# nsbuitrago/parasail-rs

Hardware: AMD Instinct MI355X
Metric: GCUPS (cell updates/s) local-affine SW, 1M 150x150 pairs, 1/2/4/8 GPUs (higher is better)
Workload: dtype int16

## Files before the change

### parasail-rs_amd/csrc/pmx_api.hip

```cpp
#include "pmx_common.h"
#include "pmx_switches.h"
#include <chrono>
#include <future>
#include "pmx_matrices.h"

#include <cctype>
#include <dlfcn.h>
#include <cstdarg>
#include <cstdio>
#include <cstdlib>
#include <cstring>
#include <algorithm>
#include <atomic>
#include <condition_variable>
#include <memory>
#include <mutex>
#include <string>
#include <system_error>
#include <thread>
#include <unordered_map>
#include <utility>
#include <vector>

static const PmxSwitchDoc g_switches[] = {
// ... 376 lines not shown
{
    if (!matrix) return;
    MatrixBox *b = nullptr;
    {
        std::lock_guard<std::mutex> lk(g_mx_mutex);
        auto it = g_boxes.find(matrix);
        if (it == g_boxes.end()) return;
        b = it->second; g_boxes.erase(it);
    }
    devcache_drop(matrix);
    delete b;
}

struct DevMat { PmxDevMatrix d; int16_t *scores; uint8_t *mapper; uint64_t hash; int rows; };
static std::mutex g_dev_mutex;
static std::unordered_map<uint64_t, DevMat> g_devmats;

static uint64_t mat_hash(const parasail_matrix_t *m)
{
    uint64_t h = 1469598103934665603ULL;
    auto mix = [&](int v) { h ^= (uint32_t)v; h *= 1099511628211ULL; };
    const size_t cells = (size_t)m->length * m->size;
    for (size_t i = 0; i < cells; ++i) mix(m->matrix[i]);
    for (int i = 0; i < 256; ++i) mix(m->mapper[i]);
    mix(m->size); mix(m->length); mix(m->type);
    return h;
}

static void devcache_drop(const parasail_matrix_t *m)
{
    std::lock_guard<std::mutex> lk(g_dev_mutex);
    for (auto it = g_devmats.begin(); it != g_devmats.end();) {
        if ((it->first >> 8) == ((uint64_t)(uintptr_t)m)) {
            (void)hipFree(it->second.scores); (void)hipFree(it->second.mapper);
            it = g_devmats.erase(it);
        } else ++it;
    }
}

static int get_devmat(const parasail_matrix_t *m, DevMat *out)
{
    if (!m || !m->matrix || !m->mapper || m->size <= 0 || m->size > 255) { set_err("bad matrix"); return -1; }
    if (m->max > 32767 || m->min < -32768) { set_err("matrix scores do not fit int16"); return -1; }
    int dev = 0; HIP_OR_RET(hipGetDevice(&dev));
    const uint64_t key = ((uint64_t)(uintptr_t)m << 8) | (uint64_t)(dev & 0xFF);
    const uint64_t h = mat_hash(m);
    std::lock_guard<std::mutex> lk(g_dev_mutex);
    auto it = g_devmats.find(key);
    if (it != g_devmats.end() && it->second.hash == h) { *out = it->second; return 0; }
    if (it != g_devmats.end()) { (void)hipFree(it->second.scores); (void)hipFree(it->second.mapper); g_devmats.erase(it); }
    const size_t cells = (size_t)m->length * m->size;
    std::vector<int16_t> s16(cells); std::vector<uint8_t> map8(256);
    for (size_t i = 0; i < cells; ++i) s16[i] = (int16_t)m->matrix[i];
    for (int i = 0; i < 256; ++i) {
        int v = m->mapper[i];
        if (v < 0 || v >= m->size) v = m->size - 1;
        map8[i] = (uint8_t)v;
    }
    DevMat dm; dm.hash = h; dm.rows = m->length;
    HIP_OR_RET(hipMalloc(&dm.scores, cells * 2));
    HIP_OR_RET(hipMalloc(&dm.mapper, 256));
    HIP_OR_RET(hipMemcpy(dm.scores, s16.data(), cells * 2, hipMemcpyHostToDevice));
    HIP_OR_RET(hipMemcpy(dm.mapper, map8.data(), 256, hipMemcpyHostToDevice));
    dm.d.scores = dm.scores; dm.d.mapper = dm.mapper; dm.d.msize = m->size; dm.d.min = m->min; dm.d.max = m->max;
    dm.d.pssm = m->type == PARASAIL_MATRIX_TYPE_PSSM ? 1 : 0; dm.d.rows = dm.d.pssm ? m->length : m->size;
    g_devmats[key] = dm;
    *out = dm;
    return 0;
}

enum {
    F_NW = 1 << 0, F_SG = 1 << 1, F_SW = 1 << 2, F_SATURATED = 1 << 6, F_BANDED = 1 << 7,
    F_SCAN = 1 << 10, F_STRIPED = 1 << 11, F_DIAG = 1 << 12, F_BLOCKED = 1 << 13,
    F_STATS = 1 << 16, F_TABLE = 1 << 17, F_ROWCOL = 1 << 18, F_TRACE = 1 << 19,
    F_BITS_8 = 1 << 20, F_BITS_16 = 1 << 21, F_BITS_32 = 1 << 22, F_BITS_64 = 1 << 23
};

struct PmxPendQueue;
struct parasail_result {
    int score, end_query, end_ref, flag;
    int matches, similar, length;
    int qlen, rlen;
    int *tables[4];
    int *rows[4];
    int *cols[4];
    int8_t *trace;
    struct PmxPendRef *pending;
};
static void pend_resolve(const parasail_result_t *r);
#define RESOLVE(r) do { if (__atomic_load_n(&(r)->pending, __ATOMIC_ACQUIRE)) pend_resolve(r); } while (0)

extern "C" {
int parasail_result_get_score(const parasail_result_t *r) { RESOLVE(r); return r->score; }
int parasail_result_get_end_query(const parasail_result_t *r) { RESOLVE(r); return r->end_query; }
int parasail_result_get_end_ref(const parasail_result_t *r) { RESOLVE(r); return r->end_ref; }
int parasail_result_get_matches(const parasail_result_t *r) { RESOLVE(r); return r->matches; }
int parasail_result_get_similar(const parasail_result_t *r) { RESOLVE(r); return r->similar; }
int parasail_result_get_length(const parasail_result_t *r) { RESOLVE(r); return r->length; }
// ... 740 lines not shown
        return "pmx_general_kernel";
    }
    if (fast_sw_eligible(cfg) && cfg->matrix->size <= PMX_MAX_FAST_MSIZE && max_qlen <= 2048 && max_rlen <= 60000)
        return "pmx_sw16_kernel";
    if ((cfg->mode == PMX_MODE_NW || cfg->mode == PMX_MODE_SG) && (cfg->want & ~PMX_WANT_SORTED) == 0 &&
        cfg->matrix->type == PARASAIL_MATRIX_TYPE_SQUARE && cfg->open >= cfg->extend && max_qlen <= 2048 &&
        cfg->matrix->size < PMX_MAX_FAST_MSIZE)
        return "pmx_nwsg16_kernel";
    if ((cfg->mode == PMX_MODE_NW || cfg->mode == PMX_MODE_SG) && (cfg->want & ~PMX_WANT_SORTED) == PMX_WANT_STATS && cfg->width != 8 &&
        cfg->matrix->type == PARASAIL_MATRIX_TYPE_SQUARE && cfg->open >= cfg->extend && cfg->extend >= 1 &&
        max_qlen <= 1024 && cfg->matrix->size < PMX_MAX_FAST_MSIZE)
        return "pmx_stats16_kernel";
    if ((cfg->want & ~PMX_WANT_SORTED) == 0 && cfg->matrix->type == PARASAIL_MATRIX_TYPE_SQUARE && cfg->matrix->size <= 64 &&
        (cfg->mode == PMX_MODE_SW || (cfg->width != 8 && cfg->width != 16)))
        return "pmx_long32_kernel";
    return "pmx_general_kernel";
}

struct Scratch { void *p = nullptr; size_t cap = 0; int dev = -1; };
enum { SCR_BOUND = 0, SCR_TRACE = 1, SCR_OPS = 2, SCR_SORT = 3, SCR_RETRY = 4,
       SCR_HQ = 5, SCR_HR = 6, SCR_HQO = 7, SCR_HRO = 8, SCR_HREC = 9, SCR_HST = 10,
       SCR_CIG = 11,
       SCR_HTEXT = 12, SCR_HTOFF = 13,
       SCR_HQ2 = 14, SCR_HR2 = 15,
       SCR_LONG = 16,
       SCR_SEL = 17,
       SCR_SRCH = 18, SCR_GREF = 19,
       SCR_PAIRS = 20, SCR_PGEN = 21,
       SCR_PUP = 22, SCR_PREC = 23, SCR_PST = 24,
       SCR_PSRCH = 25,
       SCR_PHIT = 26,
       SCR_PTOPK = 27,
       SCR_PTHIT = 28,
       SCR_SLOTS = 29 };
static thread_local Scratch g_scratch_pool[SCR_SLOTS];
static int scratch_reserve(size_t bytes, void **out, int slot = SCR_BOUND)
{
    Scratch &g_scratch = g_scratch_pool[slot];
    int dev = 0; HIP_OR_RET(hipGetDevice(&dev));
    if (g_scratch.dev != dev || g_scratch.cap < bytes) {
        if (g_scratch.p) {
            if (g_scratch.dev != dev) (void)hipSetDevice(g_scratch.dev);
            (void)hipFree(g_scratch.p);
            if (g_scratch.dev != dev) (void)hipSetDevice(dev);
        }
        g_scratch.p = nullptr; g_scratch.cap = 0; g_scratch.dev = dev;
        HIP_OR_RET(hipMalloc(&g_scratch.p, bytes ? bytes : 16));
        g_scratch.cap = bytes;
    }
    *out = g_scratch.p;
    return 0;
}

static thread_local const char *g_last_kernel = "";
extern "C" const char *pmx_last_kernel(void) { return g_last_kernel; }
static const char *nwsg_trace_kernel_name(const char *walk)
{
    static thread_local char name[160];
    snprintf(name, sizeof name, "%s%s", pmx_nwsg_trace_name(), walk);
    return name;
}


static PmxGeneralArgs general_args(const pmx_config_t *cfg, const DevMat &dm, int64_t n,
                                   const uint8_t *d_qbuf, const int64_t *d_qoff, int q_shared,
                                   const uint8_t *d_rbuf, const int64_t *d_roff, int32_t max_rlen)
{
    PmxGeneralArgs a; memset(&a, 0, sizeof a);
    a.qbuf = d_qbuf; a.qoff = q_shared ? nullptr : d_qoff; a.shared_qlen = q_shared;
    a.rbuf = d_rbuf; a.roff = d_roff; a.n = n; a.max_rlen = max_rlen;
    a.scores = dm.d.scores; a.mapper = dm.d.mapper; a.msize = dm.d.msize; a.mat_rows = dm.d.rows; a.pssm = dm.d.pssm;
    a.mode = cfg->mode; a.sg_flags = cfg->sg_flags; a.open = cfg->open; a.ext = cfg->extend;
    a.band = -1; a.bits = cfg->width;
    return a;
}

static int general_batch(const PmxGeneralArgs &t, bool want_stats, hipStream_t st, const char *what = "general kernel launch failed")
{
    const int64_t n = t.n;
    const size_t stride = (size_t)8 * t.max_rlen;
    const bool fits = pmx_general_lds_fits(t.mat_rows, t.msize, t.max_rlen);
    const size_t rs_stride = fits ? 0 : (((size_t)t.max_rlen + 8 + 15) & ~(size_t)15);
    const size_t per_pair = stride * sizeof(int32_t) + rs_stride;
// ... 402 lines not shown
                            int32_t max_qlen, int32_t max_rlen,
                            pmx_record_t *d_out, pmx_stats_t *d_stats_out, void *stream,
                            int q_shared_wild )
{
    if (check_cfg(cfg)) return -1;
    if (n <= 0) return 0;
    if (max_qlen <= 0 || max_rlen <= 0) { set_err("max_qlen / max_rlen must be positive"); return -1; }
    if ((cfg->want & PMX_WANT_STATS) && !d_stats_out) { set_err("stats requested without a stats buffer"); return -1; }
    if (cfg->want & PMX_WANT_CIGAR) { set_err("use pmx_align_batch_cigar for CIGAR output"); return -1; }
    if (pssm_batch_check(cfg->matrix, max_qlen, max_qlen)) return -1;
    DevMat dm;
    if (get_devmat(cfg->matrix, &dm)) return -1;
    hipStream_t st = (hipStream_t)stream;
    PmxBatch b = {d_qbuf, d_qoff, d_rbuf, d_roff, n, max_qlen, max_rlen, q_shared, nullptr, nullptr, nullptr, 0, 0};
    const int want = cfg->want & ~PMX_WANT_SORTED;
    if (dm.d.pssm && want == 0) { b.q_shared = max_qlen; q_shared_wild = 0; }
    if ((cfg->want & PMX_WANT_SORTED) && n >= 64 && n < (1LL << 32)) {
        void *scr = nullptr;
        if (scratch_reserve(pmx_sort_scratch_bytes(n), &scr, SCR_SORT)) return -1;
        const int rc = pmx_build_length_perm(d_roff, n, scr, &b.perm, st);
        if (rc < 0) { set_err("length sort failed (%d)", rc); return rc; }
    }
    long long long_min_cells = 250000;
    if (const char *e = pmx_env("PMX_LONG_MIN_CELLS")) long_min_cells = atoll(e);
    if (want == 0 && ((n <= 16 && max_qlen >= 512 && (long long)max_qlen * max_rlen >= long_min_cells) || max_qlen > 2048)) {
        const int rc = long_batch(cfg, dm, b, n, max_qlen, max_rlen, d_out, st);
        if (rc <= 0) return rc;
    }
    if (fast_sw_eligible(cfg)) {
        b.q_has_wildcard = b.q_shared ? q_shared_wild : 0;
        b.sat_above = cfg->width == 8 ? 127 : 0;
        if (n >= 4096 && n < (1LL << 32) && !b.q_has_wildcard) {
            void *scr = nullptr;
            if (scratch_reserve(((size_t)n + 1) * sizeof(unsigned), &scr, SCR_RETRY)) return -1;
            b.retry_count = (int *)scr;
            b.retry_list = (unsigned *)scr + 1;
        }
        const int rc = pmx_launch_sw16(b, dm.d, cfg->open, cfg->extend, d_out, st, &g_last_kernel);
        if (rc < 0) { set_err("sw16 launch failed: %s", hipGetErrorString((hipError_t)(-rc))); return rc; }
        if (rc == 0) return promote_overflowed(cfg, dm, b, d_out, st);
    }
    if (q_shared && want == PMX_WANT_STATS && cfg->width != 8 && (cfg->matrix->type == PARASAIL_MATRIX_TYPE_SQUARE || dm.d.pssm) &&
        (cfg->mode == PMX_MODE_NW || cfg->mode == PMX_MODE_SG) && (n >= 512 || pmx_env("PMX_STATS_BY_TRACE"))) {
        const int rc = stats_by_trace_shared(cfg, dm, b, d_out, d_stats_out, st);
        if (rc <= 0) return rc;
    }
    if (upload_wait(INT64_MAX, st, 0)) return -1;
    if (want == PMX_WANT_STATS && cfg->width != 8 && cfg->matrix->type == PARASAIL_MATRIX_TYPE_SQUARE) {
        auto launched = [](int rc, const char *what) {
            if (rc < 0) set_err("%s launch failed: %s", what, hipGetErrorString((hipError_t)(-rc)));
            return rc;
        };
        int rc = dm.d.msize <= 8 ? stats_by_trace_pairs(cfg, dm, b, d_out, d_stats_out, st) : 1;
        if (rc == 1)
            rc = launched(pmx_launch_stats16p(b, dm.d, cfg->mode, cfg->sg_flags, cfg->open, cfg->extend, d_out, d_stats_out, st, &g_last_kernel), "stats16p");
        if (rc == 1 && dm.d.msize > 8 && (max_rlen <= 1024 || pmx_env("PMX_STATS_BY_TRACE_ANY")))
            rc = stats_by_trace_pairs(cfg, dm, b, d_out, d_stats_out, st);
        if (rc == 1)
            rc = launched(pmx_launch_stats16(b, dm.d, cfg->mode, cfg->sg_flags, cfg->open, cfg->extend, d_out, d_stats_out, st, &g_last_kernel), "stats16");
        if (rc <= 0) return rc;
    }
    if ((cfg->mode == PMX_MODE_NW || cfg->mode == PMX_MODE_SG) && want == 0 && (cfg->width != 8 || !pmx_env("PMX_NWSG8_GENERAL")) &&
        (cfg->matrix->type == PARASAIL_MATRIX_TYPE_SQUARE || dm.d.pssm)) {
        b.track8 = cfg->width == 8;
        if (dm.d.msize <= 5 && n >= 2048 && !q_shared) {
            void *scr = nullptr;
            if (scratch_reserve(((size_t)n / 2 + 16) * sizeof(int), &scr, SCR_RETRY)) return -1;
            b.blockflag = (int *)scr;
        }
// ... 2698 lines not shown
```

### parasail-rs_amd/csrc/pmx_common.h

```cpp
#pragma once
#include <hip/hip_runtime.h>
#include <stdint.h>
#include "../../include/parasail_amd.h"
#include "../../include/pmx_conventions.h"

#define PMX_MAX_FAST_MSIZE 32

int pmx_ensure_lds_attr(const void *kernel, int bytes = 160 * 1024);

struct PmxDevMatrix {
    const int16_t *scores;
    const uint8_t *mapper;
    int msize;
    int min, max;
    int pssm;
    int rows;
};

struct PmxBatch {
    const uint8_t *qbuf; const int64_t *qoff;
    const uint8_t *rbuf; const int64_t *roff;
    int64_t n;
    int max_qlen, max_rlen;
    int q_shared;
    const unsigned *perm;
    unsigned *retry_list;
    int *retry_count;
    int q_has_wildcard;
    int sat_above;
    int track8;
    int *blockflag;
};
#define PMX_FLAG_RETRY16 4
#define PMX_FLAG_STRAND1 0x40000000

int pmx_launch_sw16(const PmxBatch &b, const PmxDevMatrix &m, int open, int ext,
                    pmx_record_t *d_out, hipStream_t stream, const char **kernel_name);

int pmx_sw16_trace_plan(const PmxBatch &b, const PmxDevMatrix &m, int open, int ext, int *variant, int *Tmax, size_t *trace_bytes);
int pmx_launch_sw16_trace(int variant, const PmxBatch &b, const PmxDevMatrix &m, int open, int ext,
                          pmx_record_t *d_out, uint32_t *tbuf, int Tmax, hipStream_t stream);

int pmx_nwsgv_bias(const PmxBatch &b, const PmxDevMatrix &m, int open, int ext, int rowx = 0, int shape_rows = 0 );
int pmx_launch_stats16p(const PmxBatch &b, const PmxDevMatrix &m, int mode, int sg_flags, int open, int ext,
                        pmx_record_t *d_out, pmx_stats_t *d_stats, hipStream_t stream, const char **kernel_name);

int pmx_nwsgv_trace_plan(const PmxBatch &b, const PmxDevMatrix &m, int mode, int open, int ext,
                         int *variant, int *Tmax, size_t *trace_bytes);
int pmx_launch_nwsgv_trace(int variant, const PmxBatch &b, const PmxDevMatrix &m, int mode, int sg_flags, int open, int ext,
                           pmx_record_t *d_out, uint32_t *tbuf, int Tmax, hipStream_t stream);
// ... 212 lines not shown
```

### parasail-rs_amd/csrc/pmx_sw16.hip

```cpp
#include "pmx_common.h"
#include "pmx_switches.h"
#include "pmx_pk16.h"
#include <cstdlib>

__device__ __forceinline__ v2s pk_adds(v2s a, v2s b) { return __builtin_elementwise_add_sat(a, b); }
__device__ __forceinline__ v2s pk_subs(v2s a, v2s b) { return __builtin_elementwise_sub_sat(a, b); }
__device__ __forceinline__ v2s pk_max(v2s a, v2s b) { return __builtin_elementwise_max(a, b); }

#ifndef PMX_SHARE_PERIOD
#define PMX_SHARE_PERIOD 16
#endif
#ifndef PMX_SW16_FUSED_HANDOFF
#define PMX_SW16_FUSED_HANDOFF 1
#endif
#define PMX_SW16_RETRY_BLOCKS 1024
#define FLOOR2 0x80008000

template <int G, int R, int VAR>
__global__ __launch_bounds__(64, (VAR == 6 && R <= 20) ? 4 : 1)
void pmx_sw16_kernel(const uint8_t *__restrict__ qbuf, const int64_t *__restrict__ qoff,
                     const uint8_t *__restrict__ rbuf, const int64_t *__restrict__ roff,
                     long long n, const int16_t *__restrict__ gmat, const uint8_t *__restrict__ gmap,
                     int msize, int open, int ext, int RP ,
                     int q_shared ,
                     int limit ,
                     const unsigned *__restrict__ perm,
                     const int *__restrict__ n_dev ,
                     unsigned *__restrict__ retry_list, int *__restrict__ retry_count ,
                     int sat_above ,
                     uint32_t *__restrict__ tbuf, int Tmax ,
                     pmx_record_t *__restrict__ out)
{
    if (n_dev) n = *n_dev;
    if ((long long)blockIdx.x * (2 * (64 / G)) >= n) return;
    constexpr bool LOOPED = VAR == 5;
    constexpr bool M3 = VAR >= 1;
    constexpr bool V2 = VAR >= 2;
    constexpr bool PT = VAR == 6;
    constexpr bool TR = VAR == 7;
    static_assert(!TR || R == 16, "trace: four packed planes of 4 rows");
    constexpr bool FETCH = VAR == 8;
    constexpr bool U8 = VAR == 3 || VAR == 5 || PT || TR || FETCH;
    constexpr bool SK = VAR >= 4;
    constexpr int EB = U8 ? 1 : 2;
    constexpr int WR = U8 ? 4 : 2;
    constexpr int RS = (R + WR - 1) / WR * WR;
    constexpr int QP = G * RS;
    constexpr int QP2 = QP / 2;
    constexpr int SLOTS = 64 / G;
    constexpr int NP = 2 * SLOTS;
    extern __shared__ __attribute__((aligned(16))) unsigned char lds[];

    long long pair0 = (long long)blockIdx.x * NP;
    do {
    int lane = threadIdx.x;
    if (LOOPED) {
        asm volatile("" : "+v"(lane));
        __syncthreads();
    }
    constexpr bool IL = G == 8 && VAR != 7;
    const int g = IL ? (lane % 16) / 2 : lane % G;
    const int slot = IL ? (lane / 16) * 2 + (lane & 1) : lane / G;
    const int PROF_STRIDE = PT ? 0 : msize * QP * EB;

    constexpr int PT_TABS = 32;
    int16_t *prof = reinterpret_cast<int16_t *>(lds);
    unsigned char *rsym = lds + (PT ? PT_TABS : NP * PROF_STRIDE + QP * EB);
    int16_t *mat = reinterpret_cast<int16_t *>(rsym + (FETCH ? 0 : NP * RP));
    unsigned char *map0 = reinterpret_cast<unsigned char *>(mat + msize * msize);
    long long *ptab = reinterpret_cast<long long *>(map0 + (PT ? 0 : 256) + ((8 - ((msize * msize * 2) & 7)) & 7));

    typedef __attribute__((address_space(3))) int *lds_int;
    auto tab_at = [](int byte) -> int { return *(lds_int)(uintptr_t)byte; };
    unsigned char *tabq = reinterpret_cast<unsigned char *>(ptab + 5 * NP);
    unsigned *wildf = reinterpret_cast<unsigned *>(tabq + 256);
    unsigned *ownmask = wildf + SLOTS;
    constexpr int OWN0 = 4 * (RS / 4 - 1), OWNN = OWN0 + R + 1;
    static_assert(!PT || OWNN <= 64, "one lane per mask");
    unsigned char *map = PT ? reinterpret_cast<unsigned char *>(ownmask + OWNN) : map0;
    static_assert(!PT || (G % 4 == 0 && RS % 4 == 0), "perm-table staging works on dwords");
    constexpr int PADF = PT ? G : G - 1;

    for (int i = lane; i < msize * msize; i += 64) mat[i] = gmat[i];
    if (PT) {
        const unsigned c4 = reinterpret_cast<const unsigned *>(gmap)[lane];
        reinterpret_cast<unsigned *>(map)[lane] = c4 << 2;
        reinterpret_cast<unsigned *>(tabq)[lane] = c4 + (c4 & 0x04040404u) * 6u;
    } else
        for (int i = lane; i < 256; i += 64) map[i] = gmap[i];
    if (PT && lane < SLOTS) wildf[lane] = 0;
    if (PT && lane < OWNN) ownmask[lane] = (unsigned)((0xFFFFFFFFull << (8 * min(max(lane - OWN0, 0), 4))) >> 32);
    if (lane < NP) {
        long long pos = pair0 + lane; if (pos >= n) pos = n - 1;
        const long long pi = perm ? (long long)perm[pos] : pos;
        const long long qb = q_shared ? 0 : qoff[pi], rb = roff[pi];
        ptab[5 * lane + 0] = qb;
        ptab[5 * lane + 1] = q_shared ? q_shared : (qoff[pi + 1] - qb);
        ptab[5 * lane + 2] = rb;
        ptab[5 * lane + 3] = roff[pi + 1] - rb;
        ptab[5 * lane + 4] = (pair0 + lane < n) ? pi : -1;
    }
    __syncthreads();
    const uint8_t *qbase = qbuf;
    const uint8_t *rbase = rbuf;

    int max_rlen = 0;
#pragma unroll
    for (int p = 0; p < NP; ++p) max_rlen = max(max_rlen, (int)ptab[5 * p + 3]);
    constexpr int UB = NP < 8 ? NP : 8;
    for (int p0 = 0; p0 < ((FETCH || PT) ? 0 : NP); p0 += UB) {
        for (int j0 = 0; j0 < RP; j0 += 64) {
            const int j = j0 + lane, jr = j - (G - 1);
            unsigned char raw[UB]; bool ok[UB];
#pragma unroll
            for (int u = 0; u < UB; ++u) {
                const int p = p0 + u;
                ok[u] = jr >= 0 && jr < (int)ptab[5 * p + 3];
                raw[u] = ok[u] ? rbase[ptab[5 * p + 2] + jr] : (unsigned char)0;
            }
            if (j < RP) {
#pragma unroll
                for (int u = 0; u < UB; ++u) {
                    const int p = p0 + u;
                    rsym[p * RP + j] = ok[u] ? map[raw[u]] : (unsigned char)((NP - p) * msize);
// ... 80 lines not shown
            const int ql = (int)ptab[5 * p + 1];
            const uint8_t *qp = qbase + ptab[5 * p + 0];
            const int p0 = 2 * rp, p1 = 2 * rp + 1;
            const int k0 = p0 % RS, k1 = p1 % RS;
            const int row0 = (p0 / RS) * R + k0, row1 = (p1 / RS) * R + k1;
            v0[u] = item < NP * QP2 && k0 < R && row0 < ql; v1[u] = item < NP * QP2 && k1 < R && row1 < ql;
            r0[u] = v0[u] ? qp[row0] : (unsigned char)0;
            r1[u] = v1[u] ? qp[row1] : (unsigned char)0;
        }
#pragma unroll
        for (int u = 0; u < QB; ++u) {
            const int item = (it0 + u) * 64 + lane;
            if (it0 + u < QITEMS && item < NP * QP2) {
                const int p = item / QP2, rp = item - p * QP2;
                const int q0 = v0[u] ? map[r0[u]] : -1;
                const int q1 = v1[u] ? map[r1[u]] : -1;
                for (int sym = 0; sym < msize; ++sym) {
                    const int s0 = ((q0 < 0) ? 0 : mat[q0 * msize + sym]) + (V2 ? open : 0);
                    const int s1 = ((q1 < 0) ? 0 : mat[q1 * msize + sym]) + (V2 ? open : 0);
                    if (U8) {
                        reinterpret_cast<unsigned short *>(lds + p * PROF_STRIDE + sym * QP)[rp] =
                            (unsigned short)((s0 & 0xFF) | ((s1 & 0xFF) << 8));
                    } else {
                        int *pp = reinterpret_cast<int *>(prof) + p * (PROF_STRIDE / 4) + rp;
                        pp[sym * QP2] = (s0 & 0xFFFF) | (s1 << 16);
                    }
                }
            }
        }
    }
    if (!PT) {
        for (int idx = lane; idx < QP * EB / 4; idx += 64)
            reinterpret_cast<int *>(lds + NP * PROF_STRIDE)[idx] = V2 ? 0 : FLOOR2;
    }
    if (PT) {
        if (lane <= msize) {
            int v = 0;
            if (lane < msize)
                for (int k = 0; k < 4 && k < msize; ++k) v |= ((mat[k * msize + lane] + open) & 0xFF) << (8 * k);
            ((lds_int)(uintptr_t)0)[lane] = v;
        }
    }
    __syncthreads();

    const int pA = 2 * slot, pB = 2 * slot + 1;
    const unsigned char *profA = lds + pA * PROF_STRIDE + g * (RS * EB);
    const unsigned char *profB = lds + pB * PROF_STRIDE + g * (RS * EB);
    constexpr int SS = PT ? 2 : 1;
    const unsigned char *rsA = PT ? rsym + slot * 2 * RP + 2 * (PADF - g) : rsym + pA * RP + (G - 1) - g;
    const unsigned char *rsB = PT ? rsA + 1 : rsym + pB * RP + (G - 1) - g;
    const int SYMSTRIDE = QP * EB;

    const v2s vOpen = PK((open & 0xFFFF) | (open << 16));
    const v2s vExt = PK((ext & 0xFFFF) | (ext << 16));
    constexpr int ZERO2 = M3 ? PK16_SW_BIAS2 : FLOOR2;
    const v2s vZero = PK(ZERO2);

    v2s HA[R], HB[R], E[R], Hsave[R];
    const int skew0 = SK ? (((G - g) * ext) & 0xFFFF) * 0x00010001 : 0;
    const v2s vC = PK(I32(vOpen) - I32(vExt));
    const v2s vInitH = V2 ? PK(ZERO2 - I32(vOpen) + skew0) : vZero;
#pragma unroll
    for (int k = 0; k < R; ++k) { HA[k] = vInitH; E[k] = V2 ? vInitH : (M3 ? PK(0) : vZero); Hsave[k] = vZero; }
    constexpr bool FUSED = SK && PMX_SW16_FUSED_HANDOFF && group_shift_fusable<G, IL>;
    if (FUSED) HB[R - 1] = PK(I32(vInitH) - I32(vExt));
    v2s best = PK(ZERO2 + skew0 - (SK ? I32(vC) : 0));
    int bestcol = g * 0x00010001;
    int vprev = 0, fake = 0;
    const int Zv0 = ZERO2 + skew0 + I32(vExt);
    const int HNEUTRAL = V2 ? ZERO2 - I32(vOpen) : ZERO2;
    int Hout = SK ? Zv0 - I32(vExt) - I32(vOpen) : HNEUTRAL, Fout = SK ? Zv0 - I32(vExt) : ZERO2;
    int Zprev = Zv0 - I32(vExt);
    int extV = I32(vExt);
    if (FUSED) asm("" : "+v"(extV));
// ... 156 lines not shown
        const v2s nbest = pk_max3(best, PK(fresh), PK(old));
        fake |= pk_lt(best, nbest);
        best = nbest;
        vprev = v;
    };
    const unsigned char *rcur = rsA;
    for (int t = 0;; t += 2) {
        if (SK && G > 1 && (t & (SHP - 1)) == 0 && t) share_bound();
        load_scores(nsA, nsB, w1a, w1b);
        if (FETCH) { nsA = symA_of(m2a); nsB = symB_of(m2b); fetch(t + 4, m2a, m2b); }
        else if (PT) { nsA = rcur[2 * SS]; nsB = rcur[2 * SS + 1]; asm("" : "+v"(nsA), "+v"(nsB)); }
        else { nsA = rsA[t + 2]; nsB = rsB[t + 2]; }
        __builtin_amdgcn_sched_barrier(0);
        step(HA, HB, w0a, w0b, t);
        __builtin_amdgcn_sched_barrier(0);
        if (t + 1 < T) {
            load_scores(nsA, nsB, w0a, w0b);
            if (FETCH) { nsA = symA_of(m3a); nsB = symB_of(m3b); fetch(t + 5, m3a, m3b); }
            else if (PT) { nsA = rcur[3 * SS]; nsB = rcur[3 * SS + 1]; asm("" : "+v"(nsA), "+v"(nsB)); rcur += 2 * SS; }
            else { nsA = rsA[t + 3]; nsB = rsB[t + 3]; }
            __builtin_amdgcn_sched_barrier(0);
            step(HB, HA, w1a, w1b, t + 1);
            __builtin_amdgcn_sched_barrier(0);
        } else
            asm("" : "=v"(Hout));
        if (t + 2 >= T) break;
    }

    unsigned long long keyA, keyB;
    {
        const int bA = (short)(I32(best) & 0xFFFF), bB = (short)(I32(best) >> 16);
        const unsigned stA = bestcol & 0xFFFF, stB = (unsigned)bestcol >> 16;
        const unsigned cA = stA - g, cB = stB - g;
        const int tA = SK ? bA - (T - (int)stA) * ext : bA, tB = SK ? bB - (T - (int)stB) * ext : bB;
        int kA = 0, kB = 0;
#pragma unroll
        for (int k = R - 1; k >= 0; --k) {
            if ((short)(I32(Hsave[k]) & 0xFFFF) == tA) kA = k;
            if ((short)(I32(Hsave[k]) >> 16) == tB) kB = k;
        }
        const int unskew = SK ? (G - g + T) * ext - (open - ext) : 0;
        const unsigned sA = (unsigned)(bA - unskew - (M3 ? PK16_SW_BIAS : -32768)), sB = (unsigned)(bB - unskew - (M3 ? PK16_SW_BIAS : -32768));
        const unsigned rA = g * R + kA, rB = g * R + kB;
        keyA = ((unsigned long long)sA << 32) | ((0xFFFFu - cA) << 16) | (0xFFFFu - rA);
        keyB = ((unsigned long long)sB << 32) | ((0xFFFFu - cB) << 16) | (0xFFFFu - rB);
        if (fake & 0xFFFF) keyA = 0;
        if (fake >> 16) keyB = 0;
    }
#pragma unroll
    for (int off = G / 2; off >= 1; off >>= 1) {
        const int lo = IL ? 2 * off : off;
        const unsigned long long oa = __shfl_xor(keyA, lo, 64), ob = __shfl_xor(keyB, lo, 64);
        keyA = oa > keyA ? oa : keyA;
        keyB = ob > keyB ? ob : keyB;
    }
    if (g == 0) {
#pragma unroll
        for (int h = 0; h < 2; ++h) {
            const long long pi = ptab[5 * (2 * slot + h) + 4];
            if (pi >= 0) {
                const unsigned long long key = h ? keyB : keyA;
                pmx_record_t rec;
                rec.score = (int)(key >> 32);
                rec.end_ref = 0xFFFF - (int)((key >> 16) & 0xFFFF);
                rec.end_query = 0xFFFF - (int)(key & 0xFFFF);
                if (M3) rec.flags = (rec.score + PK16_SW_BIAS >= limit) ? PMX_FLAG_RERUN : 0;
                else rec.flags = rec.score > 32767 ? PMX_FLAG_SATURATED : 0;
                if (rec.score > sat_above) rec.flags |= PMX_FLAG_SATURATED;
                if (PT && ((wildf[slot] >> h) & 1)) {
                    rec.flags = PMX_FLAG_RETRY16;
                    retry_list[atomicAdd(retry_count, 1)] = (unsigned)pi;
                }
                out[pi] = rec;
            }
        }
    }
    pair0 += (long long)gridDim.x * NP;
    } while (LOOPED && n_dev && pair0 < n);
}


template <int G, int R, int VAR>
static int launch_one(const PmxBatch &b, const PmxDevMatrix &m, int open, int ext,
                      pmx_record_t *d_out, hipStream_t stream, const int *n_dev = nullptr, uint32_t *tbuf = nullptr, int Tmax = 0)
{
    constexpr bool PT = VAR == 6;
    constexpr int EB = (VAR == 3 || VAR == 5 || VAR == 7 || VAR == 8 || PT) ? 1 : 2, WR = 4 / EB, RS = (R + WR - 1) / WR * WR;
    constexpr int QP = G * RS, NP = 2 * (64 / G);
    if (NP * m.msize > 255) return 1;
    const int RP = ((b.max_rlen + 2 * (G - 1) + 4 + 7) / 4) * 4;
    const size_t lds = (PT ? (size_t)256 + 4 * (64 / G) + 4 * (4 * (RS / 4 - 1) + R + 1) : (size_t)NP * m.msize * QP * EB + (size_t)QP * EB) + (VAR == 8 ? 0 : (size_t)NP * RP) +
                       (size_t)m.msize * m.msize * 2 + 256 + 8 + (size_t)NP * 40 + 32;
    if (lds > 160 * 1024) return 1;
    { const int rc = pmx_ensure_lds_attr(reinterpret_cast<const void *>(&pmx_sw16_kernel<G, R, VAR>)); if (rc) return rc; }
    long long blocks = (b.n + NP - 1) / NP;
    if (blocks <= 0) return 0;
    if (n_dev && VAR == 5 && blocks > PMX_SW16_RETRY_BLOCKS) blocks = PMX_SW16_RETRY_BLOCKS;
    if (PT) {
        hipError_t e = hipMemsetAsync(b.retry_count, 0, sizeof(int), stream);
        if (e != hipSuccess) return -(int)e;
    }
    hipLaunchKernelGGL((pmx_sw16_kernel<G, R, VAR>), dim3((unsigned)blocks), dim3(64), lds, stream,
                       b.qbuf, b.qoff, b.rbuf, b.roff, (long long)b.n, m.scores, m.mapper,
                       m.msize, open, ext, RP, b.q_shared, PK16_RERUN_LIMIT(m.max) - (VAR >= 4 ? (b.max_rlen + 2 * G + 4) * ext : 0), b.perm,
                       n_dev, b.retry_list, b.retry_count, b.sat_above > 0 ? b.sat_above : 2147483647, tbuf, Tmax, d_out);
    hipError_t e = hipGetLastError();
    if (e != hipSuccess) return -(int)e;
    if (PT) {
        PmxBatch r = b;
        r.perm = b.retry_list;
        return launch_one<G, R, 5>(r, m, open, ext, d_out, stream, b.retry_count);
    }
    return 0;
}

static bool sw16_trace_ok(const PmxBatch &b, const PmxDevMatrix &m, int open, int ext)
{
    if (pmx_env("PMX_TRACE16_GEN1") || pmx_env("PMX_SW16_NO_SKEW") || pmx_env("PMX_SW16_NO_U8") || pmx_env("PMX_SW16_VARIANT")) return false;
    if (m.msize > PMX_MAX_FAST_MSIZE || open < ext || ext < 0 || open > 1024 || b.max_rlen > 30000 || b.q_shared || b.perm) return false;
    if (m.min < -1024 || m.max > 2048 || m.min + open < 0 || open + ext > 1024 || m.max + open > 255) return false;
    const long long feasible = (long long)(b.max_qlen < b.max_rlen ? b.max_qlen : b.max_rlen) * (m.max > 0 ? m.max : 0);
    return feasible + PK16_SW_BIAS < (long long)PK16_RERUN_LIMIT(m.max) - (long long)(b.max_rlen + 2 * 64 + 4) * ext;
}
int pmx_sw16_trace_plan(const PmxBatch &b, const PmxDevMatrix &m, int open, int ext, int *variant, int *Tmax, size_t *trace_bytes)
{
    if (m.pssm) return 1;
    if (!sw16_trace_ok(b, m, open, ext)) return 1;
    if (m.msize > 8 && m.msize < 32 && !pmx_env("PMX_SW16_NO_MATRIX_LOOKUP")) {
        int G = 0;
        for (int v = 1; v < 4 && !G; ++v) if (b.max_qlen <= (8 << v) * 16) { *variant = 4 + v; G = 8 << v; }
        if (!G) return 1;
        *Tmax = (b.max_rlen + G - 1 + 1 + 15) & ~15;
        *trace_bytes = (size_t)((b.n + 2 * (64 / G) - 1) / (2 * (64 / G))) * (size_t)*Tmax * 64 * 16;
        return 0;
    }
    int G = 0;
    for (int v = 0; v < 4 && !G; ++v) {
        const int g = 8 << v, np = 2 * (64 / g);
        const size_t lds = (size_t)np * m.msize * g * 16 + (size_t)g * 16 + (size_t)np * (b.max_rlen + 2 * g + 12) +
                           (size_t)m.msize * m.msize * 2 + 256 + 8 + (size_t)np * 40 + 32;
        if (b.max_qlen <= g * 16 && np * m.msize <= 255 && lds <= 160 * 1024) { *variant = v; G = g; }
    }
    if (!G) return 1;
    const int NP = 2 * (64 / G);
// ... 4 lines not shown
int pmx_launch_sw16_trace(int variant, const PmxBatch &b, const PmxDevMatrix &m, int open, int ext,
                          pmx_record_t *d_out, uint32_t *tbuf, int Tmax, hipStream_t stream)
{
    if (m.pssm) return 1;
    if (!sw16_trace_ok(b, m, open, ext)) return 1;
    if (variant >= 4) return pmx_launch_sw16m_trace(variant - 4, b, m, open, ext, d_out, tbuf, Tmax, stream);
    switch (variant) {
    case 0: return launch_one<8, 16, 7>(b, m, open, ext, d_out, stream, nullptr, tbuf, Tmax);
    case 1: return launch_one<16, 16, 7>(b, m, open, ext, d_out, stream, nullptr, tbuf, Tmax);
    case 2: return launch_one<32, 16, 7>(b, m, open, ext, d_out, stream, nullptr, tbuf, Tmax);
    case 3: return launch_one<64, 16, 7>(b, m, open, ext, d_out, stream, nullptr, tbuf, Tmax);
    }
    return 1;
}

int pmx_launch_sw16(const PmxBatch &b, const PmxDevMatrix &m, int open, int ext,
                    pmx_record_t *d_out, hipStream_t stream, const char **kernel_name)
{
    if (m.msize > PMX_MAX_FAST_MSIZE) return 1;
    if (open < 0 || ext < 0 || open > 32767 || ext > 32767) return 1;
    if (m.max > 32767 || m.min < -32767) return 1;
    if (b.max_rlen > 60000) return 1;
    const int q = b.max_qlen;
    const char *force = pmx_env("PMX_SW16_VARIANT");
    int var = 0;
    if (open <= 1024 && ext <= 1024 && m.min >= -1024 && m.max <= 2048) var = 1;
    if (var == 1 && m.min + open >= 0 && open + ext <= 1024) var = 2;
    if (force && atoi(force) < var) var = atoi(force);
    const bool u8ok = var == 2 && m.max + open <= 255 && !pmx_env("PMX_SW16_NO_U8");
    const long long feasible = (long long)(b.max_qlen < b.max_rlen ? b.max_qlen : b.max_rlen) * (m.max > 0 ? m.max : 0);
    const bool sk = var == 2 && open >= ext && !pmx_env("PMX_SW16_NO_SKEW") &&
                    feasible + PK16_SW_BIAS < (long long)PK16_RERUN_LIMIT(m.max) - (long long)(b.max_rlen + 2 * 64 + 4) * ext;
    if (m.pssm) return (b.q_shared && var == 2 && u8ok && sk) ? pmx_launch_sw16q(b, m, open, ext, d_out, stream, kernel_name) : 1;
    const bool pt = sk && u8ok && m.msize <= 5 && b.retry_list && b.retry_count && !b.q_has_wildcard && !pmx_env("PMX_SW16_NO_PERMTABLE");
    if (b.q_shared && var == 2 && u8ok && sk && !pt) {
        const int rc = pmx_launch_sw16q(b, m, open, ext, d_out, stream, kernel_name);
        if (rc <= 0) return rc;
    }
    if (!b.q_shared && var == 2 && u8ok && sk && !pt && (m.msize > 8 || pmx_env("PMX_SW16_MATRIX_LOOKUP")) && b.n > 2048) {
        const int rc = pmx_launch_sw16m(b, m, open, ext, d_out, stream, kernel_name);
        if (rc <= 0) return rc;
    }
    const bool longref = b.max_rlen >= 1024 && !pmx_env("PMX_SW16_NO_FETCH");
#define TRY(GG, RR, NAME)                                                       \
    if (q <= (GG) * (RR)) {                                                     \
        constexpr int R4 = (RR);             \
        const bool u8 = u8ok;                                                   \
        int rc = pt ? launch_one<GG, RR, 6>(b, m, open, ext, d_out, stream)     \
               : (u8 && sk && longref) ? launch_one<GG, R4, 8>(b, m, open, ext, d_out, stream)  \
               : (u8 && sk) ? launch_one<GG, R4, 5>(b, m, open, ext, d_out, stream)  \
               : u8 ? launch_one<GG, R4, 3>(b, m, open, ext, d_out, stream)     \
               : (var == 2 && sk) ? launch_one<GG, RR, 4>(b, m, open, ext, d_out, stream)  \
               : var == 2 ? launch_one<GG, RR, 2>(b, m, open, ext, d_out, stream)  \
               : var == 1 ? launch_one<GG, RR, 1>(b, m, open, ext, d_out, stream)  \
                          : launch_one<GG, RR, 0>(b, m, open, ext, d_out, stream); \
        if (rc <= 0) { if (kernel_name) *kernel_name = pt ? NAME "/max3+vop2+skew+permtable" : var == 2 ? (sk ? ((u8 && longref) ? NAME "/max3+vop2+u8+skew+fetch" : NAME "/max3+vop2+skew") : NAME "/max3+vop2") : var == 1 ? NAME "/max3" : NAME; return rc; } \
    }
#define TRY8(RR)                                                                \
    if (u8ok && q <= 8 * (RR)) {                                                \
        int rc = pt ? launch_one<8, RR, 6>(b, m, open, ext, d_out, stream)      \
               : sk ? launch_one<8, RR, 5>(b, m, open, ext, d_out, stream) : launch_one<8, RR, 3>(b, m, open, ext, d_out, stream); \
        if (rc <= 0) { if (kernel_name) *kernel_name = pt ? "pmx_sw16_kernel<8," #RR ">/max3+vop2+skew+permtable" : sk ? "pmx_sw16_kernel<8," #RR ">/max3+vop2+u8+skew" : "pmx_sw16_kernel<8," #RR ">/max3+vop2+u8"; return rc; } \
    }
    if (b.n > 2048) { TRY8(7) TRY8(10) TRY8(13) TRY8(16) TRY8(19) TRY8(20) }
#undef TRY8
#define TRYLAT(RR)                                                              \
    if (u8ok && sk && !longref && b.n <= 64 && q <= 64 * (RR)) {                \
// ... 15 lines not shown
```

Before: 8519.

## Precompute perm-table LDS block per matrix and self-reset retry counter in kernel

Builds the perm-table staging block (mapper tables, wildcard flags, ownership masks, open-biased score tables) once per matrix, open and tile shape in a small setup kernel, caches it on the device matrix, and has each block copy it into LDS instead of recomputing it. The retry counter moves to its own scratch slot and the last retiring block of the retry kernel zeroes it, which removes the per-call hipMemsetAsync. The best-row search after the DP also switches to packed u16 min/mad instructions. The cost is extra cached device state per matrix plus a one-time synchronizing setup launch, and correctness now depends on the in-kernel reset staying in step across calls.

```diff
diff --git a/parasail-rs_amd/csrc/pmx_api.hip b/parasail-rs_amd/csrc/pmx_api.hip
--- a/parasail-rs_amd/csrc/pmx_api.hip
+++ b/parasail-rs_amd/csrc/pmx_api.hip
@@ -432,7 +432,7 @@
     std::lock_guard<std::mutex> lk(g_dev_mutex);
     for (auto it = g_devmats.begin(); it != g_devmats.end();) {
         if ((it->first >> 8) == ((uint64_t)(uintptr_t)m)) {
-            (void)hipFree(it->second.scores); (void)hipFree(it->second.mapper);
+            (void)hipFree(it->second.scores); (void)hipFree(it->second.mapper); pmx_sw16_tabs_free(it->second.d.sw16_tabs);
             it = g_devmats.erase(it);
         } else ++it;
     }
@@ -448,7 +448,7 @@
     std::lock_guard<std::mutex> lk(g_dev_mutex);
     auto it = g_devmats.find(key);
     if (it != g_devmats.end() && it->second.hash == h) { *out = it->second; return 0; }
-    if (it != g_devmats.end()) { (void)hipFree(it->second.scores); (void)hipFree(it->second.mapper); g_devmats.erase(it); }
+    if (it != g_devmats.end()) { (void)hipFree(it->second.scores); (void)hipFree(it->second.mapper); pmx_sw16_tabs_free(it->second.d.sw16_tabs); g_devmats.erase(it); }
     const size_t cells = (size_t)m->length * m->size;
     std::vector<int16_t> s16(cells); std::vector<uint8_t> map8(256);
     for (size_t i = 0; i < cells; ++i) s16[i] = (int16_t)m->matrix[i];
@@ -464,6 +464,7 @@
     HIP_OR_RET(hipMemcpy(dm.mapper, map8.data(), 256, hipMemcpyHostToDevice));
     dm.d.scores = dm.scores; dm.d.mapper = dm.mapper; dm.d.msize = m->size; dm.d.min = m->min; dm.d.max = m->max;
     dm.d.pssm = m->type == PARASAIL_MATRIX_TYPE_PSSM ? 1 : 0; dm.d.rows = dm.d.pssm ? m->length : m->size;
+    dm.d.sw16_tabs = pmx_sw16_tabs_new();
     g_devmats[key] = dm;
     *out = dm;
     return 0;
@@ -1270,7 +1271,8 @@
        SCR_PHIT = 26,
        SCR_PTOPK = 27,
        SCR_PTHIT = 28,
-       SCR_SLOTS = 29 };
+       SCR_RETRYCNT = 29,
+       SCR_SLOTS = 30 };
 static thread_local Scratch g_scratch_pool[SCR_SLOTS];
 static int scratch_reserve(size_t bytes, void **out, int slot = SCR_BOUND)
 {
@@ -1287,6 +1289,18 @@
         g_scratch.cap = bytes;
     }
     *out = g_scratch.p;
+    return 0;
+}
+
+static int retry_counter(int **out)
+{
+    const Scratch &s = g_scratch_pool[SCR_RETRYCNT];
+    int dev = 0; HIP_OR_RET(hipGetDevice(&dev));
+    const bool fresh = s.dev != dev || s.cap < 2 * sizeof(int);
+    void *p = nullptr;
+    if (scratch_reserve(2 * sizeof(int), &p, SCR_RETRYCNT)) return -1;
+    if (fresh) { HIP_OR_RET(hipMemset(p, 0, 2 * sizeof(int))); HIP_OR_RET(hipStreamSynchronize(nullptr)); }
+    *out = (int *)p;
     return 0;
 }
 
@@ -1755,9 +1769,9 @@
         b.sat_above = cfg->width == 8 ? 127 : 0;
         if (n >= 4096 && n < (1LL << 32) && !b.q_has_wildcard) {
             void *scr = nullptr;
-            if (scratch_reserve(((size_t)n + 1) * sizeof(unsigned), &scr, SCR_RETRY)) return -1;
-            b.retry_count = (int *)scr;
-            b.retry_list = (unsigned *)scr + 1;
+            if (scratch_reserve((size_t)n * sizeof(unsigned), &scr, SCR_RETRY)) return -1;
+            b.retry_list = (unsigned *)scr;
+            if (retry_counter(&b.retry_count)) return -1;
         }
         const int rc = pmx_launch_sw16(b, dm.d, cfg->open, cfg->extend, d_out, st, &g_last_kernel);
         if (rc < 0) { set_err("sw16 launch failed: %s", hipGetErrorString((hipError_t)(-rc))); return rc; }
diff --git a/parasail-rs_amd/csrc/pmx_common.h b/parasail-rs_amd/csrc/pmx_common.h
--- a/parasail-rs_amd/csrc/pmx_common.h
+++ b/parasail-rs_amd/csrc/pmx_common.h
@@ -15,7 +15,10 @@
     int min, max;
     int pssm;
     int rows;
-};
+    struct PmxSw16Tabs *sw16_tabs;
+};
+struct PmxSw16Tabs *pmx_sw16_tabs_new();
+void pmx_sw16_tabs_free(struct PmxSw16Tabs *t);
 
 struct PmxBatch {
     const uint8_t *qbuf; const int64_t *qoff;
diff --git a/parasail-rs_amd/csrc/pmx_sw16.hip b/parasail-rs_amd/csrc/pmx_sw16.hip
--- a/parasail-rs_amd/csrc/pmx_sw16.hip
+++ b/parasail-rs_amd/csrc/pmx_sw16.hip
@@ -2,6 +2,8 @@
 #include "pmx_switches.h"
 #include "pmx_pk16.h"
 #include <cstdlib>
+#include <mutex>
+#include <vector>
 
 __device__ __forceinline__ v2s pk_adds(v2s a, v2s b) { return __builtin_elementwise_add_sat(a, b); }
 __device__ __forceinline__ v2s pk_subs(v2s a, v2s b) { return __builtin_elementwise_sub_sat(a, b); }
@@ -16,11 +18,34 @@
 #define PMX_SW16_RETRY_BLOCKS 1024
 #define FLOOR2 0x80008000
 
+constexpr int pmx_sw16_pt_own0(int R) { return 4 * ((R + 3) / 4 - 1); }
+constexpr int pmx_sw16_pt_tail_dwords(int G, int R) { return 64 + 64 / G + pmx_sw16_pt_own0(R) + R + 1 + 64; }
+constexpr int PMX_SW16_PT_TABS = 32;
+
+__global__ __launch_bounds__(64)
+void pmx_sw16_tables_kernel(const int16_t *__restrict__ gmat, const uint8_t *__restrict__ gmap, int msize, int open,
+                            int slots, int own0, int R, unsigned *__restrict__ block)
+{
+    const int lane = threadIdx.x, ownn = own0 + R + 1;
+    const unsigned c4 = reinterpret_cast<const unsigned *>(gmap)[lane];
+    block[lane] = c4 + (c4 & 0x04040404u) * 6u;
+    if (lane < slots) block[64 + lane] = 0;
+    if (lane < ownn) block[64 + slots + lane] = (unsigned)((0xFFFFFFFFull << (8 * min(max(lane - own0, 0), 4))) >> 32);
+    block[64 + slots + ownn + lane] = c4 << 2;
+    if (lane < PMX_SW16_PT_TABS / 4) {
+        int v = 0;
+        if (lane < msize)
+            for (int k = 0; k < 4 && k < msize; ++k) v |= ((gmat[k * msize + lane] + open) & 0xFF) << (8 * k);
+        block[128 + slots + ownn + lane] = v;
+    }
+}
+
 template <int G, int R, int VAR>
 __global__ __launch_bounds__(64, (VAR == 6 && R <= 20) ? 4 : 1)
 void pmx_sw16_kernel(const uint8_t *__restrict__ qbuf, const int64_t *__restrict__ qoff,
                      const uint8_t *__restrict__ rbuf, const int64_t *__restrict__ roff,
                      long long n, const int16_t *__restrict__ gmat, const uint8_t *__restrict__ gmap,
+                     const unsigned *__restrict__ pt_block ,
                      int msize, int open, int ext, int RP ,
                      int q_shared ,
                      int limit ,
@@ -32,7 +57,13 @@
                      pmx_record_t *__restrict__ out)
 {
     if (n_dev) n = *n_dev;
-    if ((long long)blockIdx.x * (2 * (64 / G)) >= n) return;
+    auto retire = [&]() {
+        if (VAR == 5 && n_dev && threadIdx.x == 0 && atomicAdd(retry_count + 1, 1) == (int)gridDim.x - 1) {
+            retry_count[0] = 0;
+            retry_count[1] = 0;
+        }
+    };
+    if ((long long)blockIdx.x * (2 * (64 / G)) >= n) { retire(); return; }
     constexpr bool LOOPED = VAR == 5;
     constexpr bool M3 = VAR >= 1;
     constexpr bool V2 = VAR >= 2;
@@ -63,7 +94,7 @@
     const int slot = IL ? (lane / 16) * 2 + (lane & 1) : lane / G;
     const int PROF_STRIDE = PT ? 0 : msize * QP * EB;
 
-    constexpr int PT_TABS = 32;
+    constexpr int PT_TABS = PMX_SW16_PT_TABS;
     int16_t *prof = reinterpret_cast<int16_t *>(lds);
     unsigned char *rsym = lds + (PT ? PT_TABS : NP * PROF_STRIDE + QP * EB);
     int16_t *mat = reinterpret_cast<int16_t *>(rsym + (FETCH ? 0 : NP * RP));
@@ -77,19 +108,23 @@
     unsigned *ownmask = wildf + SLOTS;
     constexpr int OWN0 = 4 * (RS / 4 - 1), OWNN = OWN0 + R + 1;
     static_assert(!PT || OWNN <= 64, "one lane per mask");
+    static_assert(OWN0 == pmx_sw16_pt_own0(R) || !PT, "the block's layout is the carve's");
     unsigned char *map = PT ? reinterpret_cast<unsigned char *>(ownmask + OWNN) : map0;
     static_assert(!PT || (G % 4 == 0 && RS % 4 == 0), "perm-table staging works on dwords");
     constexpr int PADF = PT ? G : G - 1;
 
-    for (int i = lane; i < msize * msize; i += 64) mat[i] = gmat[i];
-    if (PT) {
-        const unsigned c4 = reinterpret_cast<const unsigned *>(gmap)[lane];
-        reinterpret_cast<unsigned *>(map)[lane] = c4 << 2;
-        reinterpret_cast<unsigned *>(tabq)[lane] = c4 + (c4 & 0x04040404u) * 6u;
-    } else
+    if constexpr (PT) {
+        constexpr int NT = pmx_sw16_pt_tail_dwords(G, R), NB = NT + PT_TABS / 4;
+#pragma unroll
+        for (int i0 = 0; i0 < NB; i0 += 64) {
+            const int i = i0 + lane;
+            if (i0 + 64 <= NT) reinterpret_cast<unsigned *>(tabq)[i] = pt_block[i];
+            else if (i < NB) *(i < NT ? reinterpret_cast<unsigned *>(tabq) + i : reinterpret_cast<unsigned *>(lds) + (i - NT)) = pt_block[i];
+        }
+    } else {
+        for (int i = lane; i < msize * msize; i += 64) mat[i] = gmat[i];
         for (int i = lane; i < 256; i += 64) map[i] = gmap[i];
-    if (PT && lane < SLOTS) wildf[lane] = 0;
-    if (PT && lane < OWNN) ownmask[lane] = (unsigned)((0xFFFFFFFFull << (8 * min(max(lane - OWN0, 0), 4))) >> 32);
+    }
     if (lane < NP) {
         long long pos = pair0 + lane; if (pos >= n) pos = n - 1;
         const long long pi = perm ? (long long)perm[pos] : pos;
@@ -236,14 +271,6 @@
     if (!PT) {
         for (int idx = lane; idx < QP * EB / 4; idx += 64)
             reinterpret_cast<int *>(lds + NP * PROF_STRIDE)[idx] = V2 ? 0 : FLOOR2;
-    }
-    if (PT) {
-        if (lane <= msize) {
-            int v = 0;
-            if (lane < msize)
-                for (int k = 0; k < 4 && k < msize; ++k) v |= ((mat[k * msize + lane] + open) & 0xFF) << (8 * k);
-            ((lds_int)(uintptr_t)0)[lane] = v;
-        }
     }
     __syncthreads();
 
@@ -466,13 +493,17 @@
         const int bA = (short)(I32(best) & 0xFFFF), bB = (short)(I32(best) >> 16);
         const unsigned stA = bestcol & 0xFFFF, stB = (unsigned)bestcol >> 16;
         const unsigned cA = stA - g, cB = stB - g;
-        const int tA = SK ? bA - (T - (int)stA) * ext : bA, tB = SK ? bB - (T - (int)stB) * ext : bB;
-        int kA = 0, kB = 0;
+        const v2us T2 = {(unsigned short)T, (unsigned short)T};
+        const v2us tgt2 = SK ? __builtin_bit_cast(v2us, best) - (T2 - __builtin_bit_cast(v2us, bestcol)) * __builtin_bit_cast(v2us, vExt)
+                             : __builtin_bit_cast(v2us, best);
+        int acc = (int)((unsigned)(-R & 0xFFFF) * 0x00010001u);
 #pragma unroll
         for (int k = R - 1; k >= 0; --k) {
-            if ((short)(I32(Hsave[k]) & 0xFFFF) == tA) kA = k;
-            if ((short)(I32(Hsave[k]) >> 16) == tB) kB = k;
-        }
+            int y;
+            asm("v_pk_min_u16 %0, %1, %2" : "=v"(y) : "v"(I32(Hsave[k]) ^ __builtin_bit_cast(int, tgt2)), "s"(0x00010001));
+            asm("v_pk_mad_u16 %0, %1, %0, %1" : "+v"(acc) : "v"(y));
+        }
+        const int kA = acc & 0xFFFF, kB = (unsigned)acc >> 16;
         const int unskew = SK ? (G - g + T) * ext - (open - ext) : 0;
         const unsigned sA = (unsigned)(bA - unskew - (M3 ? PK16_SW_BIAS : -32768)), sB = (unsigned)(bB - unskew - (M3 ? PK16_SW_BIAS : -32768));
         const unsigned rA = g * R + kA, rB = g * R + kB;
@@ -511,8 +542,40 @@
     }
     pair0 += (long long)gridDim.x * NP;
     } while (LOOPED && n_dev && pair0 < n);
-}
-
+    retire();
+}
+
+
+struct PmxSw16Tabs {
+    struct Entry { int open, G, R; unsigned *block; };
+    std::mutex mu;
+    std::vector<Entry> entries;
+};
+PmxSw16Tabs *pmx_sw16_tabs_new() { return new PmxSw16Tabs; }
+void pmx_sw16_tabs_free(PmxSw16Tabs *t)
+{
+    if (!t) return;
+    for (auto &e : t->entries) (void)hipFree(e.block);
+    delete t;
+}
+static int sw16_pt_block(const PmxDevMatrix &m, int open, int G, int R, hipStream_t stream, const unsigned **out)
+{
+    PmxSw16Tabs *t = m.sw16_tabs;
+    std::lock_guard<std::mutex> lk(t->mu);
+    for (auto &e : t->entries)
+        if (e.open == open && e.G == G && e.R == R) { *out = e.block; return 0; }
+    unsigned *block = nullptr;
+    hipError_t e = hipMalloc(&block, (size_t)(pmx_sw16_pt_tail_dwords(G, R) + PMX_SW16_PT_TABS / 4) * sizeof(unsigned));
+    if (e != hipSuccess) return -(int)e;
+    hipLaunchKernelGGL(pmx_sw16_tables_kernel, dim3(1), dim3(64), 0, stream, m.scores, m.mapper, m.msize, open, 64 / G,
+                       pmx_sw16_pt_own0(R), R, block);
+    e = hipGetLastError();
+    if (e == hipSuccess) e = hipStreamSynchronize(stream);
+    if (e != hipSuccess) { (void)hipFree(block); return -(int)e; }
+    t->entries.push_back({open, G, R, block});
+    *out = block;
+    return 0;
+}
 
 template <int G, int R, int VAR>
 static int launch_one(const PmxBatch &b, const PmxDevMatrix &m, int open, int ext,
@@ -530,12 +593,10 @@
     long long blocks = (b.n + NP - 1) / NP;
     if (blocks <= 0) return 0;
     if (n_dev && VAR == 5 && blocks > PMX_SW16_RETRY_BLOCKS) blocks = PMX_SW16_RETRY_BLOCKS;
-    if (PT) {
-        hipError_t e = hipMemsetAsync(b.retry_count, 0, sizeof(int), stream);
-        if (e != hipSuccess) return -(int)e;
-    }
+    const unsigned *pt_block = nullptr;
+    if (PT) { const int rc = sw16_pt_block(m, open, G, R, stream, &pt_block); if (rc) return rc; }
     hipLaunchKernelGGL((pmx_sw16_kernel<G, R, VAR>), dim3((unsigned)blocks), dim3(64), lds, stream,
-                       b.qbuf, b.qoff, b.rbuf, b.roff, (long long)b.n, m.scores, m.mapper,
+                       b.qbuf, b.qoff, b.rbuf, b.roff, (long long)b.n, m.scores, m.mapper, pt_block,
                        m.msize, open, ext, RP, b.q_shared, PK16_RERUN_LIMIT(m.max) - (VAR >= 4 ? (b.max_rlen + 2 * G + 4) * ext : 0), b.perm,
                        n_dev, b.retry_list, b.retry_count, b.sat_above > 0 ? b.sat_above : 2147483647, tbuf, Tmax, d_out);
     hipError_t e = hipGetLastError();
@@ -543,7 +604,9 @@
     if (PT) {
         PmxBatch r = b;
         r.perm = b.retry_list;
-        return launch_one<G, R, 5>(r, m, open, ext, d_out, stream, b.retry_count);
+        const int rc = launch_one<G, R, 5>(r, m, open, ext, d_out, stream, b.retry_count);
+        if (rc) (void)hipMemsetAsync(b.retry_count, 0, 2 * sizeof(int), stream);
+        return rc;
     }
     return 0;
 }
@@ -614,7 +677,7 @@
     const bool sk = var == 2 && open >= ext && !pmx_env("PMX_SW16_NO_SKEW") &&
                     feasible + PK16_SW_BIAS < (long long)PK16_RERUN_LIMIT(m.max) - (long long)(b.max_rlen + 2 * 64 + 4) * ext;
     if (m.pssm) return (b.q_shared && var == 2 && u8ok && sk) ? pmx_launch_sw16q(b, m, open, ext, d_out, stream, kernel_name) : 1;
-    const bool pt = sk && u8ok && m.msize <= 5 && b.retry_list && b.retry_count && !b.q_has_wildcard && !pmx_env("PMX_SW16_NO_PERMTABLE");
+    const bool pt = sk && u8ok && m.msize <= 5 && m.sw16_tabs && b.retry_list && b.retry_count && !b.q_has_wildcard && !pmx_env("PMX_SW16_NO_PERMTABLE");
     if (b.q_shared && var == 2 && u8ok && sk && !pt) {
         const int rc = pmx_launch_sw16q(b, m, open, ext, d_out, stream, kernel_name);
         if (rc <= 0) return rc;
```

After: 8519. No clear change (-0.0%).
